# LIS-TU-Berlin/SVN-ICP

Measured on NVIDIA B200. Metric: scans/sec at 1000 particles (64-beam ~120k-pt synthetic scan, K=100, 30 SVN iterations), higher is better.
Workload: dtype f32 geometry / f64 reduction+Stein

## Files before the change

include/svnicp_b200.h:

```cpp
#ifndef SVNICP_B200_H
#define SVNICP_B200_H

#include <stdint.h>

#ifdef __cplusplus
extern "C" {
#endif

#define SVNICP_B200_ABI_VERSION 2

typedef struct svnicp_handle_t *svnicp_handle;

typedef enum {
  SVNICP_OK = 0,
  SVNICP_ERR_INVALID = -1,
  SVNICP_ERR_NO_DEVICE = -2,
  SVNICP_ERR_CUDA = -3,
  SVNICP_ERR_NCCL = -4,
  SVNICP_ERR_OOM = -5
} svnicp_status;

#define SVNICP_ALIGN_SUCCESS 1
#define SVNICP_NO_OPTIMIZER 2

#define SVNICP_CLASS_SVNICP 0
#define SVNICP_CLASS_SVGDICP 1

typedef struct {
  int32_t iterations;
  int32_t use_minibatch;
  int32_t batch_size;
  double lr;
  double max_dist;
  int32_t normalize_cloud;
  char optimizer[16];
  int32_t check_early_stop;
  int32_t convergence_steps;
  double convergence_threshold;
  int32_t KNN_count;
  int32_t SVN_full_grad;
  int32_t use_weight_mean;
  double grid_cell;
  int32_t debug_corr;
  int32_t flags;
  int32_t gn_stages;
  int32_t gn_smem_kb;
} svnicp_params;

#define SVNICP_FLAG_NO_PARTICLE_SORT 1
#define SVNICP_FLAG_FILTER_FULL 2
#define SVNICP_FLAG_NCCL_GATHER 8
#define SVNICP_FLAG_DEBUG_SYNC 32
#define SVNICP_FLAG_WATCHDOG 64
#define SVNICP_FLAG_NO_GRAPH 128
#define SVNICP_FLAG_FORCE_GRAPH 256
#define SVNICP_FLAG_REUSE_STATS 16

void svnicp_default_params(svnicp_params *p);

int svnicp_abi_version(void);

int svnicp_create(svnicp_handle *out, const svnicp_params *params, int particle_count, const double *init_pose,
                  int class_type, int device);
void svnicp_destroy(svnicp_handle h);
const char *svnicp_last_error(svnicp_handle h);

int svnicp_set_stream(svnicp_handle h, void *cuda_stream);

int svnicp_nccl_unique_id(void *id128);
int svnicp_init_sharding(svnicp_handle h, const void *unique_id128, int rank, int n_ranks);

int svnicp_add_cloud(svnicp_handle h, const double *source, int64_t n_s, int source_on_device, const double *target,
                     int64_t n_t, int target_on_device, const double *init_pose);

int svnicp_set_initial_mean(svnicp_handle h, const double R0[9], const double t0[3]);

int svnicp_align(svnicp_handle h);

int svnicp_get_transformation(svnicp_handle h, double out6[6]);
int svnicp_get_distribution(svnicp_handle h, double out6[6]);
int svnicp_get_cov_matrix(svnicp_handle h, double out36[36]);
int svnicp_get_particles(svnicp_handle h, double *out_6xP);
int svnicp_get_particle_weight(svnicp_handle h, double *out_P);
int svnicp_get_particle_history(svnicp_handle h, float *out_Ix6xP, int32_t *rows );
int svnicp_get_runtime(svnicp_handle h, double out3[3]);
int svnicp_set_k(svnicp_handle h, int k);
int svnicp_set_threshold(svnicp_handle h, double max_dist);

int svnicp_initialize_particles(int particle_count, const double ub[6], const double lb[6], uint64_t seed, double *out_6xP);
int svnicp_initialize_particles_gaussian(int particle_count, const double cov_diag[6], uint64_t seed, double *out_6xP);

int svnicp_iterations_done(svnicp_handle h, int32_t *out);
int svnicp_get_candidates(svnicp_handle h, int32_t *out_idx , float *out_rel_xyz );
int svnicp_get_source_f32(svnicp_handle h, float *out_xyz);
int svnicp_get_correspondences(svnicp_handle h, float *out_transforms, int32_t *out_idx, uint8_t *out_mask);
int svnicp_get_gn_system(svnicp_handle h, double *out_H, double *out_b, double *out_x);
int svnicp_get_stein(svnicp_handle h, double *out_delta, double *out_bandwidth);
int svnicp_get_prune_stats(svnicp_handle h, double *out_mean_kept, int32_t *rows);
int svnicp_get_timing(svnicp_handle h, double out4[4]);
int svnicp_get_slice(svnicp_handle h, int32_t *lo, int32_t *hi);
int svnicp_set_profiling(svnicp_handle h, int on);
int svnicp_get_phase_times(svnicp_handle h, double out8[8]);
int svnicp_get_scan_info(svnicp_handle h, int64_t out8[8]);
int svnicp_get_tail_stamps(svnicp_handle h, double out8[8]);
int svnicp_get_launch_count(svnicp_handle h, int64_t *out);

typedef struct svnicp_batch_t *svnicp_batch;
int svnicp_batch_create(svnicp_batch *out, const svnicp_params *params, int n_streams, int particle_count, const double *init_pose,
                        int device);
// ... 36 lines not shown
```

svn_icp_b200/__init__.py:

```python
from __future__ import annotations

import ctypes as C
import dataclasses
import os

import numpy as np

_HERE = os.path.dirname(os.path.abspath(__file__))
LIB_PATH = os.environ.get("SVNICP_B200_LIB") or os.path.join(_HERE, "lib", "libsvnicp_b200.so")

ALIGN_SUCCESS = 1
NO_OPTIMIZER = 2
CLASS_SVNICP = 0
CLASS_SVGDICP = 1


class SvnIcpError(RuntimeError):
    pass


class _CParams(C.Structure):
    _fields_ = [("iterations", C.c_int32), ("use_minibatch", C.c_int32), ("batch_size", C.c_int32), ("lr", C.c_double),
                ("max_dist", C.c_double), ("normalize_cloud", C.c_int32), ("optimizer", C.c_char * 16),
                ("check_early_stop", C.c_int32), ("convergence_steps", C.c_int32), ("convergence_threshold", C.c_double),
                ("KNN_count", C.c_int32), ("SVN_full_grad", C.c_int32), ("use_weight_mean", C.c_int32),
                ("grid_cell", C.c_double), ("debug_corr", C.c_int32), ("flags", C.c_int32), ("gn_stages", C.c_int32),
                ("gn_smem_kb", C.c_int32)]


FLAG_NO_PARTICLE_SORT = 1
FLAG_FILTER_FULL = 2
FLAG_NCCL_GATHER = 8
FLAG_REUSE_STATS = 16
FLAG_DEBUG_SYNC = 32
FLAG_WATCHDOG = 64
FLAG_NO_GRAPH = 128
FLAG_FORCE_GRAPH = 256


@dataclasses.dataclass
class SteinICPParam:
    iterations: int = 50
    use_minibatch: bool = False
    batch_size: int = 50
    lr: float = 0.02
    max_dist: float = 1.0
    normalize_cloud: bool = True
    optimizer: str = "Adam"
    check_early_stop: bool = False
    convergence_steps: int = 5
    convergence_threshold: float = 1e-5
    KNN_count: int = 100
    SVN_full_grad: bool = True
    grid_cell: float = 0.0
    debug_corr: bool = False
    flags: int = 0
    gn_stages: int = 0
    gn_smem_kb: int = 0


@dataclasses.dataclass
class ParticleWeightOpt:
    use_weight_mean: bool = False


_lib = None

EXPORTS = [
    "svnicp_abi_version", "svnicp_default_params", "svnicp_create", "svnicp_destroy", "svnicp_last_error", "svnicp_set_stream",
    "svnicp_nccl_unique_id", "svnicp_init_sharding", "svnicp_add_cloud", "svnicp_set_initial_mean", "svnicp_align",
    "svnicp_get_transformation", "svnicp_get_distribution", "svnicp_get_cov_matrix", "svnicp_get_particles",
    "svnicp_get_particle_weight", "svnicp_get_particle_history", "svnicp_get_runtime", "svnicp_set_k", "svnicp_set_threshold",
    "svnicp_initialize_particles", "svnicp_initialize_particles_gaussian", "svnicp_iterations_done", "svnicp_get_candidates",
    "svnicp_get_source_f32", "svnicp_get_correspondences", "svnicp_get_gn_system", "svnicp_get_stein", "svnicp_get_prune_stats",
    "svnicp_get_timing", "svnicp_get_slice", "svnicp_get_launch_count", "svnicp_set_profiling", "svnicp_get_phase_times",
    "svnicp_get_scan_info", "svnicp_get_tail_stamps",
    "svnicp_map_create", "svnicp_map_destroy", "svnicp_map_last_error", "svnicp_map_clear", "svnicp_map_add_cloud", "svnicp_map_get",
    "svnicp_map_download", "svnicp_map_size",
    "svnicp_pre_create", "svnicp_pre_destroy", "svnicp_pre_last_error", "svnicp_pre_crop", "svnicp_pre_downsample_uniform",
    "svnicp_pre_to_f64", "svnicp_pre_download", "svnicp_pre_deskew", "svnicp_pose_compose",
    "svnicp_batch_create", "svnicp_batch_destroy", "svnicp_batch_last_error", "svnicp_batch_size", "svnicp_batch_stream", "svnicp_batch_align",
]


def load_library() -> C.CDLL:
    global _lib
    if _lib is None:
        if not os.path.exists(LIB_PATH):
            raise SvnIcpError(f"{LIB_PATH} not found: build it with `python -m svn_icp_b200.build` "
                              "(there is no CPU or PyTorch fallback for this path)")
# ... 498 lines not shown
```

svn_icp_b200/csrc/cand_build.cu:

```cuda
#include "common.cuh"
#include "kernels.h"

namespace svn {

constexpr unsigned long long EMPTY_KEY = 0xffffffffffffffffull;
constexpr int RING_MAX = 6;
constexpr int KNN_WARPS = 4;
#ifndef SVN_KNN_CAP
#define SVN_KNN_CAP 512
#endif
constexpr int KNN_CAP = SVN_KNN_CAP;
constexpr int KNN_BINS = 64;

struct Ent {
  double d;
  int pos;
  int idx;
};

__device__ __forceinline__ int cell_of(double x, double inv_cell) { return (int)floor(x * inv_cell); }
__device__ __forceinline__ unsigned long long pack_key(int cx, int cy, int cz) {
  return ((unsigned long long)(unsigned)(cx + (1 << 20)) & 0x1fffffull) << 42 |
         ((unsigned long long)(unsigned)(cy + (1 << 20)) & 0x1fffffull) << 21 |
         ((unsigned long long)(unsigned)(cz + (1 << 20)) & 0x1fffffull);
// ... 322 lines not shown
        SVN_KNN_RELIEVE()
      }
    }
#undef SVN_KNN_RELIEVE
    if (done) {
      int *hist = s_hist[warp];
      hist[lane] = 0;
      hist[lane + 32] = 0;
      __syncwarp();
      const double scale = (double)KNN_BINS / rs2_done;
      for (int i = lane; i < count; i += 32) {
        const double d = buf[i].d;
        if (d < rs2_done) atomicAdd(&hist[min(KNN_BINS - 1, (int)(d * scale))], 1);
      }
      __syncwarp();
      const int h0 = hist[2 * lane], h1 = hist[2 * lane + 1];
      int incl = h0 + h1;
#pragma unroll
      for (int o = 1; o < 32; o <<= 1) {
        const int v = __shfl_up_sync(0xffffffffu, incl, o);
        if (lane >= o) incl += v;
      }
      const int before = incl - h0 - h1;
      int tbin = KNN_BINS;
      if (before < K && before + h0 >= K) tbin = 2 * lane;
      else if (before + h0 < K && incl >= K) tbin = 2 * lane + 1;
#pragma unroll
      for (int o = 16; o > 0; o >>= 1) tbin = min(tbin, __shfl_xor_sync(0xffffffffu, tbin, o));
      int m_out = 0;
      for (int i0 = 0; i0 < count; i0 += 32) {
        const int i = i0 + lane;
        Ent e;
        bool keep = false;
        if (i < count) {
          e = buf[i];
          keep = (e.d < rs2_done) && (min(KNN_BINS - 1, (int)(e.d * scale)) <= tbin);
        }
        const unsigned m = __ballot_sync(0xffffffffu, keep);
        __syncwarp();
        if (keep) buf[m_out + __popc(m & lt_mask)] = e;
        m_out += __popc(m);
        __syncwarp();
      }
      count = m_out;
    }
    count = warp_compact(buf, count, K, &tau);

    for (int k = lane; k < K; k += 32) {
      const double *m;
      int gi;
      if (k < count) { m = sxyz + 3 * (size_t)buf[k].pos; gi = buf[k].idx; }
      else { m = tgt; gi = 0; }
      const float cx = __double2float_rn(m[0] - q[0]), cy = __double2float_rn(m[1] - q[1]), cz = __double2float_rn(m[2] - q[2]);
      const double nrm = sqrt((double)cx * cx + (double)cy * cy + (double)cz * cz);
      const float w = (k < count) ? __double2float_rd(nrm * (1.0 - 1e-6)) : INFINITY;
      cand[(size_t)b * K + k] = make_float4(cx, cy, cz, w);
      if (cand_idx) cand_idx[(size_t)b * K + k] = gi;
    }
    __syncwarp();
  }
}

static inline int cdiv(long long a, long long b) { return (int)((a + b - 1) / b); }

size_t knn_smem_bytes() { return (size_t)KNN_WARPS * KNN_CAP * sizeof(Ent); }

int launch_cand_build(const CandBuildArgs &a, cudaStream_t st) {
  int launches = 0;
  const int T = 256;
  k_q0<<<cdiv(a.n_pad, T), T, 0, st>>>(a.src64, a.n_s, a.sc, a.q0, a.sp, a.n_pad); launches++;
  k_grid_clear<<<cdiv(a.table_size, T), T, 0, st>>>(a.keys, a.counts, a.fill, a.table_size, a.cursor); launches++;
  k_grid_count<<<cdiv(a.n_t, T), T, 0, st>>>(a.tgt64, a.n_t, 1.0 / a.cell, a.keys, a.counts, a.pt_slot, (unsigned)(a.table_size - 1)); launches++;
  k_grid_alloc<<<cdiv(a.table_size, T), T, 0, st>>>(a.counts, a.starts, a.table_size, a.cursor); launches++;
  k_grid_scatter<<<cdiv(a.n_t, T), T, 0, st>>>(a.tgt64, a.n_t, a.pt_slot, a.starts, a.fill, a.sxyz, a.sidx); launches++;
  if (knn_smem_bytes() > 48 * 1024) cudaFuncSetAttribute(k_knn, cudaFuncAttributeMaxDynamicSharedMemorySize, (int)knn_smem_bytes());
  int grid = cdiv(a.row_hi - a.row_lo, KNN_WARPS);
  const int max_grid = a.sm_count * 12;
  if (grid > max_grid) grid = max_grid;
  if (grid < 1) grid = 1;
  k_knn<<<grid, KNN_WARPS * 32, knn_smem_bytes(), st>>>(a.q0, a.row_lo, a.row_hi, a.tgt64, a.n_t, a.sxyz, a.sidx, a.keys, a.starts, a.counts,
                                                         (unsigned)(a.table_size - 1), a.cell, a.K, a.cand, a.cand_idx, a.fallback_count);
  launches++;
  return launches;
}

}
```

svn_icp_b200/csrc/capi.cu:

```cuda
#include <cuda_runtime.h>
#include <dlfcn.h>
#include <math.h>
#include <nccl.h>
#include <stdarg.h>
#include <stdio.h>
#include <time.h>
#include <stdlib.h>
#include <string.h>

#include <algorithm>
#include <cmath>
#include <string>
#include <vector>

#include "../../include/svnicp_b200.h"
#include "common.cuh"
#include "kernels.h"

using namespace svn;

static thread_local std::string g_create_error;

struct NcclApi {
  void *lib = nullptr;
// ... 666 lines not shown
    h->launches += launch_stats_svgd(sa0, nullptr, st);
    CU(cudaGetLastError());
    CU(cudaMemcpyAsync(h->h_stats, h->stats.p, 48 * sizeof(double), cudaMemcpyDeviceToHost, st));
    CU(cudaMemcpyAsync(h->h_particles, h->particles.p, (size_t)6 * h->P * sizeof(double), cudaMemcpyDeviceToHost, st));
    CU(cudaStreamSynchronize(st));
    memset(h->h_ctrl, 0, sizeof(Ctrl));
    memset(h->h_kept, 0, ((size_t)I + 2) * sizeof(unsigned long long));
    h->iters_done = 0;
    h->enqueued_iters = 0;
    h->ms_setup = h->ms_iter = h->ms_epi = h->ms_total = 0;
    h->aligned = true;
    S.special = true;
    return SVNICP_NO_OPTIMIZER;
  }

  CU(cudaEventRecord(h->ev[0], st));
  CandBuildArgs cb;
  cb.src64 = h->src64.p; cb.tgt64 = h->tgt64.p;
  cb.n_s = (int)h->n_s; cb.n_pad = h->n_pad; cb.n_t = (int)h->n_t; cb.K = h->K;
  cb.sc = h->sc;
  cb.cell = h->prm.grid_cell > 0 ? h->prm.grid_cell : 1.5;
  cb.q0 = h->q0.p; cb.sp = h->sp.p;
  cb.keys = h->keys.p; cb.counts = h->counts.p; cb.starts = h->starts.p; cb.fill = h->fill.p; cb.pt_slot = h->pt_slot.p;
  cb.cursor = h->misc.p; cb.fallback_count = h->misc.p + 1;
  size_t table = 1024;
  while (table < (size_t)2 * h->n_t) table <<= 1;
  cb.table_size = (int)table;
  cb.sxyz = h->sxyz.p; cb.sidx = h->sidx.p; cb.cand = h->cand.p; cb.cand_idx = h->prm.debug_corr ? h->cand_idx.p : nullptr;
  cb.sm_count = h->sm_count;
  cb.row_lo = h->rank * h->rows_per_rank;
  cb.row_hi = cb.row_lo + h->rows_per_rank < (int)h->n_s ? cb.row_lo + h->rows_per_rank : (int)h->n_s;
  if (cb.row_hi < cb.row_lo) cb.row_hi = cb.row_lo;
  h->launches += launch_cand_build(cb, st);
  if (h->n_ranks > 1) {
    const size_t blk = (size_t)h->rows_per_rank * h->K;
    NC(g_nccl.AllGather(h->cand.p + (size_t)h->rank * blk, h->cand.p, blk * 4, ncclFloat, h->comm, st));
    if (h->prm.debug_corr) NC(g_nccl.AllGather(h->cand_idx.p + (size_t)h->rank * blk, h->cand_idx.p, blk, ncclInt32, h->comm, st));
  }
  CU(cudaGetLastError());
  CU(cudaEventRecord(h->ev[1], st));

  IterArgs &ia = S.ia;
  memset(&ia, 0, sizeof(ia));
  ia.n_s = (int)h->n_s; ia.n_pad = h->n_pad; ia.K = h->K; ia.Kp = h->Kp; ia.cand_idx = h->prm.debug_corr ? h->cand_idx.p : nullptr;
  ia.P = h->P; ia.p_lo = h->p_lo; ia.P_l = h->P_l;
  ia.sc = h->sc;
  ia.max_dist = (float)h->max_dist;
  ia.sp = h->sp.p; ia.cand = h->cand.p; ia.clist = h->clist.p; ia.hdr = h->hdr.p;
  ia.R = h->R.p; ia.t = h->t.p; ia.xf = h->xf.p; ia.dnorm = h->dnorm.p; ia.part = h->part.p; ia.rec = h->rec; ia.rec_stride = h->rec_stride; ia.ctrl = h->ctrl.p;
  ia.TB = h->TB; ia.stages = h->stages; ia.n_slices = h->n_slices; ia.n_pgroups = h->n_pgroups; ia.PG = h->PG; ia.RG = h->RG;
  ia.gn_lag = (h->prm.gn_stages >> 8) ? (h->prm.gn_stages >> 8) : ((h->stages >= 4) ? 2 : 1);
  ia.gn_smem = h->gn_smem; ia.sm_count = h->sm_count; ia.svn_full_grad = h->prm.SVN_full_grad;
  ia.first_order = svgd ? 1 : 0;
  ia.dbg_idx = h->prm.debug_corr ? h->dbg_idx.p : nullptr;
  ia.dbg_mask = h->prm.debug_corr ? h->dbg_mask.p : nullptr;

  SteinArgs &sa = S.sa;
  memset(&sa, 0, sizeof(sa));
  sa.P = h->P; sa.p_lo = h->p_lo; sa.P_l = h->P_l; sa.I = I;
  sa.svn_full_grad = h->prm.SVN_full_grad; sa.check_early_stop = h->prm.check_early_stop;
  sa.lr = h->prm.lr; sa.threshold = h->prm.convergence_threshold;
  sa.rec = h->rec; sa.rec_stride = h->rec_stride; sa.xs = h->xs.p; sa.delta = h->delta.p; sa.dnorm = h->dnorm.p; sa.R = h->R.p; sa.t = h->t.p;
  sa.Hbar_inv = h->Hbar_inv.p; sa.hist = h->hist.p; sa.history = h->history.p; sa.ctrl = h->ctrl.p;
  sa.stats = h->stats.p; sa.particles = h->particles.p; sa.sm_count = h->sm_count;
  sa.kept_hist = h->kept_hist.p;
  sa.prep_scratch_d = h->prep_scratch_d.p;
  sa.prep_scratch_i = h->prep_scratch_i.p;
  sa.stamps = h->profile ? h->stamps.p : nullptr;
  const bool overlap = S.overlap = !svgd && (h->n_ranks == 1 || h->peer_mode);
  S.pt = h->pt;
  S.seq0 = h->seq;
  S.use_graph = overlap && h->n_ranks == 1 && !h->profile && !h->prm.debug_corr && !h->graph_off &&
                !(h->prm.flags & (SVNICP_FLAG_DEBUG_SYNC | SVNICP_FLAG_NO_GRAPH)) &&
                ((h->prm.flags & SVNICP_FLAG_FORCE_GRAPH) || (!h->prm.check_early_stop && I >= 16 && (double)h->n_s * (double)h->P_l <= 1.0e7));

  if (h->profile)
    while (h->prof_events.size() < (size_t)I * 7) {
      cudaEvent_t pe;
      CU(cudaEventCreate(&pe));
      h->prof_events.push_back(pe);
    }
  if (!svgd) {
    const double *x_src = (realign && h->n_ranks > 1) ? h->rec + (size_t)(h->iters_done & 1) * h->rec_stride : nullptr;
    h->launches += launch_prep(ia, st, 1, x_src);
    if (overlap) CU(cudaEventRecord(h->ev_x, st));
  }
  S.e = 0;
  S.enqueue_done = I <= 0;
  return SVNICP_OK;
}

static int align_step(svnicp_handle h, AlignState &S) {
  ALIGN_LOCALS
  const int LAG = 3;
  const int e = S.e;
    if (h->prm.check_early_stop && e >= LAG) {
      CU(cudaEventSynchronize(h->iter_events[e - LAG]));
      if (h->h_stop[e - LAG]) { S.enqueue_done = true; return SVNICP_OK; }
    }
#define PROF(k)                                                                                          \
  do {                                                                                                   \
    if (h->profile) CU(cudaEventRecord(h->prof_events[(size_t)e * 7 + (k)], st));                        \
    if (h->prm.flags & SVNICP_FLAG_DEBUG_SYNC) {                                                         \
      fprintf(stderr, "[svnicp] iteration %d: before phase %d ...", e, (k));                             \
      fflush(stderr);                                                                                    \
      const cudaError_t e1__ = cudaStreamSynchronize(st), e2__ = cudaStreamSynchronize(hs);              \
// ... 532 lines not shown
```

svn_icp_b200/csrc/iter_kernels.cu:

```cuda
#include "common.cuh"
#include "kernels.h"
#include "ptx.cuh"

namespace svn {

__global__ void __launch_bounds__(1024) k_prep(IterArgs a, int all_x, const double *x_src) {
  if (a.ctrl->stop) return;
  __shared__ double s_red[32][12];
  __shared__ float s_center[12];
  __shared__ double s_max[32][2];
  __shared__ int s_env[PRUNE_BINS];
  __shared__ int s_nan;
  const int tid = threadIdx.x, lane = tid & 31, warp = tid >> 5;
  const double *R0 = a.sc.R0;
  double acc[12];
#pragma unroll
  for (int i = 0; i < 12; i++) acc[i] = 0.0;
  for (int l = tid; l < a.P_l; l += blockDim.x) {
    const int p = a.p_lo + l;
    double R[9], t[3], w[3];
#pragma unroll
    for (int i = 0; i < 9; i++) R[i] = a.R[9 * (size_t)p + i];
#pragma unroll
    for (int i = 0; i < 3; i++) t[i] = a.t[3 * (size_t)p + i];
// ... 319 lines not shown
__device__ __forceinline__ float sqrt_approx(float x) {
  float r;
  asm("sqrt.approx.ftz.f32 %0, %1;" : "=f"(r) : "f"(x));
  return r;
}
__device__ __forceinline__ float rcp_approx(float x) {
  float r;
  asm("rcp.approx.ftz.f32 %0, %1;" : "=f"(r) : "f"(x));
  return r;
}

typedef unsigned long long f2;
__device__ __forceinline__ f2 pk(float a, float b) { f2 r; asm("mov.b64 %0, {%1, %2};" : "=l"(r) : "f"(a), "f"(b)); return r; }
__device__ __forceinline__ float lo(f2 v) { float a; asm("{ .reg .f32 t; mov.b64 {%0, t}, %1; }" : "=f"(a) : "l"(v)); return a; }
__device__ __forceinline__ float hi(f2 v) { float a; asm("{ .reg .f32 t; mov.b64 {t, %0}, %1; }" : "=f"(a) : "l"(v)); return a; }
__device__ __forceinline__ f2 bc(float s) { return pk(s, s); }
__device__ __forceinline__ f2 fma2(f2 a, f2 b, f2 c) { f2 r; asm("fma.rn.f32x2 %0, %1, %2, %3;" : "=l"(r) : "l"(a), "l"(b), "l"(c)); return r; }
__device__ __forceinline__ f2 add2(f2 a, f2 b) { f2 r; asm("add.rn.f32x2 %0, %1, %2;" : "=l"(r) : "l"(a), "l"(b)); return r; }
__device__ __forceinline__ f2 sub2(f2 a, f2 b) { f2 r; asm("sub.rn.f32x2 %0, %1, %2;" : "=l"(r) : "l"(a), "l"(b)); return r; }
__device__ __forceinline__ f2 mul2(f2 a, f2 b) { f2 r; asm("mul.rn.f32x2 %0, %1, %2;" : "=l"(r) : "l"(a), "l"(b)); return r; }
__device__ __forceinline__ f2 neg2(f2 a) { return pk(-lo(a), -hi(a)); }
__device__ __forceinline__ f2 sel2(bool p0, bool p1, f2 a, f2 b) { return pk(p0 ? lo(a) : lo(b), p1 ? hi(a) : hi(b)); }
__device__ __forceinline__ f2 min4_2(f2 a, f2 b, f2 c, f2 d) {
  return pk(fminf(fminf(lo(a), lo(b)), fminf(lo(c), lo(d))), fminf(fminf(hi(a), hi(b)), fminf(hi(c), hi(d))));
}

__device__ __noinline__ void gn_dbg_tap(const IterArgs &a, int row, int l, float qx, float qy, float qz, float ex, float ey, float ez, bool valid) {
  const float4 *full_row = a.cand + (size_t)row * a.K;
  const float wx_ = __fsub_rn(qx, ex), wy_ = __fsub_rn(qy, ey), wz_ = __fsub_rn(qz, ez);
  int slot = 0;
  float bd_ = INFINITY;
  for (int kk = 0; kk < a.K; kk++) {
    const float4 f = full_row[kk];
    const float dd_ = fabsf(f.x - wx_) + fabsf(f.y - wy_) + fabsf(f.z - wz_);
    if (dd_ < bd_) { bd_ = dd_; slot = kk; }
  }
  a.dbg_idx[(size_t)l * a.n_s + row] = a.cand_idx[(size_t)row * a.K + slot];
  a.dbg_mask[(size_t)l * a.n_s + row] = valid ? 1 : 0;
}

__device__ __forceinline__ void gn_recover(const float4 *e, int bk, float qx, float qy, float qz, float best, float &ex, float &ey, float &ez) {
  const float4 c0 = e[bk], c1 = e[bk + 1], c2 = e[bk + 2], c3 = e[bk + 3];
#define SVN_D1(C, T)                                                                                      \
  const float T##x = __fsub_rn(qx, (C).x), T##y = __fsub_rn(qy, (C).y), T##z = __fsub_rn(qz, (C).z);       \
  const float T##d = __fmaf_rn(T##z, T##z, __fmaf_rn(T##y, T##y, __fmul_rn(T##x, T##x)));
  SVN_D1(c0, u) SVN_D1(c1, v) SVN_D1(c2, w) SVN_D1(c3, z)
#undef SVN_D1
  (void)zd;
  const bool h0 = ud == best, h1 = vd == best, h2 = wd == best;
  ex = h0 ? ux : h1 ? vx : h2 ? wx : zx;
  ey = h0 ? uy : h1 ? vy : h2 ? wy : zy;
  ez = h0 ? uz : h1 ? vz : h2 ? wz : zz;
  if (best == INFINITY) { ex = ux; ey = uy; ez = uz; }
}

template <bool DBG, bool UNI, bool FIRST>
__global__ void __launch_bounds__(GN_THREADS, 1) k_gn(IterArgs a) {
  if (a.ctrl->stop) return;
  extern __shared__ __align__(128) unsigned char smem[];
  const int TB = a.TB, Kp = a.Kp, S = a.stages;
  const size_t stage_bytes = gn_stage_bytes(TB, Kp);
  uint64_t *full = reinterpret_cast<uint64_t *>(smem + (size_t)S * stage_bytes);
  uint64_t *empty = full + S;
  const int tid = threadIdx.x, warp = tid >> 5, lane = tid & 31;
  const int n_tiles = a.n_pad / TB;
  const int slice = blockIdx.x, n_slices = gridDim.x;
  const int n_my = (slice < n_tiles) ? (n_tiles - slice + n_slices - 1) / n_slices : 0;
  const size_t hdr_off = (size_t)TB * Kp * 16, msk_off = hdr_off + (size_t)TB * 16;

  if (tid == 0) {
    for (int s = 0; s < S; s++) { mbar_init(full + s, 1); mbar_init(empty + s, GN_CONSUMERS / 32); }
    fence_barrier_init();
  }
  __syncthreads();

  constexpr int NW = GN_CONSUMERS / 32;
  auto tile_cnt = [&](int j) -> int {
    return (lane < TB) ? (__float_as_int(__ldg(&a.hdr[(size_t)(slice + j * n_slices) * TB + lane].w)) >> 16) : 0;
  };
  auto tile_issue = [&](int j, int cnt) {
    const int s = j % S;
    const int row0 = (slice + j * n_slices) * TB;
    unsigned char *st = smem + (size_t)s * stage_bytes;
    const unsigned m2 = __ballot_sync(0xffffffffu, cnt == 2), m4 = __ballot_sync(0xffffffffu, cnt == 4), ml = __ballot_sync(0xffffffffu, cnt > 4);
    const int bytes = cnt * 16;
    SVN_CHECK(a.ctrl, cnt >= 0 && cnt <= Kp && row0 + TB <= a.n_pad, 1);
    int total = bytes;
#pragma unroll
    for (int o = 16; o > 0; o >>= 1) total += __shfl_xor_sync(0xffffffffu, total, o);
    total += TB * 16;
    if (lane == 0) {
      unsigned *msk = reinterpret_cast<unsigned *>(st + msk_off);
      msk[0] = m2; msk[1] = m4; msk[2] = ml;
      mbar_expect_tx(full + s, (uint32_t)total);
    }
    __syncwarp();
    if (lane < TB && cnt > 0) bulk_g2s(st + (size_t)lane * Kp * 16, a.clist + (size_t)(row0 + lane) * Kp, (uint32_t)bytes, full + s);
    if (lane == 0) bulk_g2s(st + hdr_off, a.hdr + row0, (uint32_t)(TB * 16), full + s);
  };
  const int LAG = (a.gn_lag < S) ? a.gn_lag : 1, AHEAD = S - LAG;
  for (int j = 0; j < AHEAD && j < n_my; j++)
    if (warp == j % NW) tile_issue(j, tile_cnt(j));
  int cnt_pref = (warp == 0 && AHEAD < n_my) ? tile_cnt(AHEAD) : 0;

  const int PG = a.PG, RG = a.RG;
  const int pl = tid % PG, rg = tid / PG;
// ... 80 lines not shown
      unsigned m2 = msk[0] & rgmask, m4 = msk[1] & rgmask, ml = msk[2] & rgmask;
      rows_in_acc += __popc(m2 | m4 | ml);
#define SVN_ROW2(SV, CA, CB)                                                                                            \
  {                                                                                                                     \
    const float4 sv = (SV);                                                                                             \
    SVN_QUERY                                                                                                           \
    SVN_DIST(CA, u) SVN_DIST(CB, v)                                                                                     \
                                 \
    const bool p0 = lo(vd) < lo(ud), p1 = hi(vd) < hi(ud);                                                              \
    const f2 best = sel2(p0, p1, vd, ud), ex = sel2(p0, p1, vx, ux), ey = sel2(p0, p1, vy, uy), ez = sel2(p0, p1, vz, uz); \
    SVN_ACCUM(true)                                                                                                     \
  }
      while (m2 & (m2 - 1)) {
        const int r0 = __ffs(m2) - 1;
        m2 &= m2 - 1;
        const int r1 = __ffs(m2) - 1;
        m2 &= m2 - 1;
        const float4 sv0 = hdr[r0], sv1 = hdr[r1];
        const float4 *e0 = lists + r0 * Kp, *e1 = lists + r1 * Kp;
        const float4 c00 = e0[0], c01 = e0[1], c10 = e1[0], c11 = e1[1];
        { const int r = r0; (void)r; SVN_ROW2(sv0, c00, c01) }
        { const int r = r1; (void)r; SVN_ROW2(sv1, c10, c11) }
      }
      if (m2) {
        const int r = __ffs(m2) - 1;
        const float4 *e0 = lists + r * Kp;
        const float4 sv0 = hdr[r], c00 = e0[0], c01 = e0[1];
        SVN_ROW2(sv0, c00, c01)
      }
#undef SVN_ROW2
      while (m4) {
        const int r = __ffs(m4) - 1;
        m4 &= m4 - 1;
        const float4 sv = hdr[r];
        const float4 *e = lists + r * Kp;
        const float4 c0 = e[0], c1 = e[1], c2 = e[2], c3 = e[3];
        SVN_QUERY
        SVN_DIST(c0, u) SVN_DIST(c1, v) SVN_DIST(c2, w) SVN_DIST(c3, z)
        const bool p10 = lo(vd) < lo(ud), p11 = hi(vd) < hi(ud), p30 = lo(zd) < lo(wd), p31 = hi(zd) < hi(wd);
        const f2 m01 = sel2(p10, p11, vd, ud), m23 = sel2(p30, p31, zd, wd);
        const f2 e01x = sel2(p10, p11, vx, ux), e01y = sel2(p10, p11, vy, uy), e01z = sel2(p10, p11, vz, uz);
        const f2 e23x = sel2(p30, p31, zx, wx), e23y = sel2(p30, p31, zy, wy), e23z = sel2(p30, p31, zz, wz);
        const bool p0 = lo(m23) < lo(m01), p1 = hi(m23) < hi(m01);
        const f2 best = sel2(p0, p1, m23, m01), ex = sel2(p0, p1, e23x, e01x), ey = sel2(p0, p1, e23y, e01y), ez = sel2(p0, p1, e23z, e01z);
        SVN_ACCUM(true)
      }
      while (ml) {
        const int r = __ffs(ml) - 1;
        ml &= ml - 1;
        const float4 sv = hdr[r];
        const float4 *e = lists + r * Kp;
        const int n = __float_as_int(sv.w) >> 16;
        SVN_CHECK(a.ctrl, n > 4 && n <= Kp && (n & 3) == 0 && r < TB, 2);
        float4 c0 = e[0], c1 = e[1], c2 = e[2], c3 = e[3];
        SVN_QUERY
        float best0, best1;
        int bk0 = 0, bk1 = 0;
        {
          SVN_DIST(c0, u) SVN_DIST(c1, v) SVN_DIST(c2, w) SVN_DIST(c3, z)
          const f2 m_ = min4_2(ud, vd, wd, zd);
          best0 = lo(m_); best1 = hi(m_);
          if (!(best0 == best0)) best0 = INFINITY;
          if (!(best1 == best1)) best1 = INFINITY;
        }
        const f2 qq = fma2(qz, qz, fma2(qy, qy, mul2(qx, qx)));
        const f2 qn = fma2(pk(sqrt_approx(lo(qq)), sqrt_approx(hi(qq))), bc(1.00001f), bc(1e-7f));
        for (int k0 = 4; k0 < n; k0 += 4) {
          c0 = e[k0]; c1 = e[k0 + 1]; c2 = e[k0 + 2]; c3 = e[k0 + 3];
          const f2 tt = sub2(bc(c0.w), qn);
          const f2 tb = mul2(mul2(tt, tt), bc(0.99999f));
          const bool done = (lo(tt) > 0.f) && (lo(tb) > best0) && (hi(tt) > 0.f) && (hi(tb) > best1);
          if (UNI) { if (__all_sync(0xffffffffu, done)) break; }
          else { if (done) break; }
          SVN_DIST(c0, u) SVN_DIST(c1, v) SVN_DIST(c2, w) SVN_DIST(c3, z)
          const f2 m_ = min4_2(ud, vd, wd, zd);
          if (lo(m_) < best0) { best0 = lo(m_); bk0 = k0; }
          if (hi(m_) < best1) { best1 = hi(m_); bk1 = k0; }
        }
        SVN_CHECK(a.ctrl, bk0 >= 0 && bk0 + 3 < n && bk1 >= 0 && bk1 + 3 < n, 3);
        float ex0, ey0, ez0, ex1, ey1, ez1;
        gn_recover(e, bk0, lo(qx), lo(qy), lo(qz), best0, ex0, ey0, ez0);
        gn_recover(e, bk1, hi(qx), hi(qy), hi(qz), best1, ex1, ey1, ez1);
        const f2 best = pk(best0, best1), ex = pk(ex0, ex1), ey = pk(ey0, ey1), ez = pk(ez0, ez1);
        SVN_ACCUM(true)
      }
      if (rows_in_acc >= GN_FLUSH_ROWS) {
#pragma unroll
        for (int j = 0; j < NACC; j++) { dacc[j * GN_CONSUMERS] = add2(dacc[j * GN_CONSUMERS], acc[j]); acc[j] = 0; }
        rows_in_acc = 0;
        if (++flushes2 >= GN_FLUSH2 && active) {
#pragma unroll
          for (int j = 0; j < NACC; j++) {
            const f2 d = dacc[j * GN_CONSUMERS];
            out[j] = (wrote ? out[j] : 0.0) + (double)lo(d);
            if (active1) out[NACC + j] = (wrote ? out[NACC + j] : 0.0) + (double)hi(d);
            dacc[j * GN_CONSUMERS] = 0;
          }
          wrote = true;
          flushes2 = 0;
        }
      }
    }
    __syncwarp();
    if (lane == 0) mbar_arrive(empty + s);
  }
#undef SVN_QUERY
#undef SVN_DIST
#undef SVN_ACCUM
  if (active) {
#pragma unroll
    for (int j = 0; j < NACC; j++) {
      const f2 d = dacc[j * GN_CONSUMERS];
      out[j] = (wrote ? out[j] : 0.0) + ((double)lo(d) + (double)lo(acc[j]));
      if (active1) out[NACC + j] = (wrote ? out[NACC + j] : 0.0) + ((double)hi(d) + (double)hi(acc[j]));
    }
  }
}

__global__ void __launch_bounds__(FIN_WARPS * 32) k_finalize(IterArgs a, PeerTable pt, unsigned seq_h) {
  Ctrl *ctl = a.ctrl;
  if (ctl->stop) return;
  __shared__ double s_out[REC];
  __shared__ int s_last;
  const int l = blockIdx.x;
  double v[NACC];
  gn_sum_partials(a, l, v);
  const int p = a.p_lo + l;
  SVN_CHECK(ctl, l < a.P_l && p < a.P && (size_t)(p + 1) * REC <= a.rec_stride, 20);
  const size_t buf_off = (size_t)(ctl->iter & 1) * a.rec_stride;
  if (threadIdx.x == 0) {
    const double *R0 = a.sc.R0;
    double Rp[9], Rt[9];
#pragma unroll
    for (int i = 0; i < 9; i++) Rp[i] = a.R[9 * (size_t)p + i];
#pragma unroll
// ... 144 lines not shown
```

svn_icp_b200/csrc/kernels.h:

```cpp
#pragma once
#include <cuda_runtime.h>
#include <stdint.h>
#include "common.cuh"

namespace svn {

struct CandBuildArgs {
  const double *src64, *tgt64;
  int n_s, n_pad, n_t, K;
  int row_lo, row_hi;
  ScanConst sc;
  double cell;
  double *q0;
  float4 *sp;
  unsigned long long *keys;
  int *counts, *starts, *fill, *pt_slot, *cursor;
  int table_size;
  double *sxyz;
  int *sidx;
  float4 *cand;
  int *cand_idx;
  int *fallback_count;
  int sm_count;
};
int launch_cand_build(const CandBuildArgs &a, cudaStream_t st);
size_t knn_smem_bytes();

struct IterArgs {
  int n_s, n_pad, K;
  int Kp;
  const int *cand_idx;
  int P;
  int p_lo, P_l;
  ScanConst sc;
  float max_dist;
  const float4 *sp, *cand;
  float4 *clist;
  float4 *hdr;
  const float4 *clist_prev;
  const int *cbase_prev;
  const float4 *ball_prev;
  int *cbase;
  float4 *ball;
  const unsigned long long *kept_hist;
  double *R, *t;
  float *xf;
  double *dnorm;
  double *part;
  double *rec;
  size_t rec_stride;
  Ctrl *ctrl;
  int TB, stages, n_slices, n_pgroups, PG, RG;
  int gn_lag;
  size_t gn_smem;
  int sm_count;
  int svn_full_grad;
  int first_order;
  int32_t *dbg_idx;
  uint8_t *dbg_mask;
};
#ifdef __CUDACC__
constexpr int FIN_WARPS = 8;
__host__ __device__ inline int fin_rows(const IterArgs &a) { return a.n_slices * (a.RG < a.TB ? a.RG : a.TB); }
inline int fin_threads(const IterArgs &a) { return fin_rows(a) > 512 ? FIN_WARPS * 32 : 128; }
__device__ __forceinline__ void gn_sum_partials(const IterArgs &a, int l, double v[NACC]) {
  __shared__ double s_fin[FIN_WARPS][NACC];
  const int lane = threadIdx.x & 31, w = threadIdx.x >> 5, nw = blockDim.x >> 5;
  const int nrows = fin_rows(a);
  const int j16 = lane & 15, half = lane >> 4;
  double s0 = 0.0, s1 = 0.0, s2 = 0.0, s3 = 0.0;
  const int step = 2 * nw;
  int r = half + 2 * w;
  for (; r + 3 * step < nrows; r += 4 * step) {
    s0 += a.part[((size_t)r * a.P_l + l) * NACC + j16];
    s1 += a.part[((size_t)(r + step) * a.P_l + l) * NACC + j16];
    s2 += a.part[((size_t)(r + 2 * step) * a.P_l + l) * NACC + j16];
    s3 += a.part[((size_t)(r + 3 * step) * a.P_l + l) * NACC + j16];
  }
  for (; r < nrows; r += step) s0 += a.part[((size_t)r * a.P_l + l) * NACC + j16];
  double s = (s0 + s1) + (s2 + s3);
  s += __shfl_down_sync(0xffffffffu, s, 16);
  if (lane < NACC) s_fin[w][lane] = s;
  __syncthreads();
#pragma unroll
  for (int j = 0; j < NACC; j++) {
    double t = s_fin[0][j];
    for (int ww = 1; ww < nw; ww++) t += s_fin[ww][j];
    v[j] = t;
  }
}
#endif
int launch_prep(const IterArgs &a, cudaStream_t st, int all_x, const double *x_src);
int launch_filter(const IterArgs &a, cudaStream_t st);
int launch_gn(const IterArgs &a, cudaStream_t st);
int launch_finalize(const IterArgs &a, const PeerTable &pt, unsigned seq_h, cudaStream_t st);
void init_iter_kernels();
__host__ __device__ inline size_t gn_stage_bytes(int TB, int K) { return ((size_t)TB * K * 16 + (size_t)TB * 16 + 16 + 127) & ~(size_t)127; }
constexpr int GN_CONSUMERS = 512;
constexpr int GN_THREADS = GN_CONSUMERS;
__host__ __device__ inline size_t gn_dacc_offset(int TB, int K, int S) { return (gn_stage_bytes(TB, K) * S + 2 * (size_t)S * 8 + 127) & ~(size_t)127; }
__host__ __device__ inline size_t gn_smem_bytes(int TB, int K, int S) { return gn_dacc_offset(TB, K, S) + (size_t)NACC * GN_CONSUMERS * 8; }

struct SteinArgs {
  int P, p_lo, P_l, I;
  int svn_full_grad, check_early_stop;
  double lr, threshold;
  double *rec;
  size_t rec_stride;
  double *xs;
  double *delta;
  double *dnorm;
  double *R, *t;
  double *Hbar_inv;
  unsigned *hist;
  float *history;
  Ctrl *ctrl;
  double *stats;
  double *particles;
  unsigned long long *kept_hist;
  double *prep_scratch_d;
  int *prep_scratch_i;
  double *stamps;
  int sm_count;
};
int launch_head(const SteinArgs &a, const PeerTable &pt, unsigned seq_x, int epilogue, cudaStream_t st);
int launch_tail(const SteinArgs &a, const IterArgs &ia, const PeerTable &pt, unsigned seq_h, unsigned seq_x_out, cudaStream_t st);
int launch_decide(const SteinArgs &a, cudaStream_t st, int epilogue);
int launch_median(const SteinArgs &a, cudaStream_t st);
int launch_stats(const SteinArgs &a, int parity_from_ctrl, cudaStream_t st);
int launch_align_reset(Ctrl *ctrl, double *opt_state, size_t n_opt, cudaStream_t st);
int launch_init_particles(double *R, double *t, const double *init_pose_dev, int P, double *dnorm, int p_lo, int P_l, Ctrl *ctrl,
                          cudaStream_t st);


enum { SVGD_OPT_ADAM = 0, SVGD_OPT_RMSPROP = 1, SVGD_OPT_SGD = 2, SVGD_OPT_ADAGRAD = 3 };
struct SvgdArgs {
  int P, p_lo, P_l;
  int optimizer;
  double lr;
  double *pose6;
  double *prev;
  double *opt_state;
};
int launch_svgd_init(const SvgdArgs &s, const double *init_pose_dev, double *R, double *t, double *dnorm, Ctrl *ctrl, cudaStream_t st);
int launch_finalize_first(const IterArgs &a, const SvgdArgs &s, cudaStream_t st);
int launch_svgd_rec(double *rec, const double *src6, const double *dnorm, int lo, int n, int dn_off, cudaStream_t st);
int launch_stein_first(const SteinArgs &a, cudaStream_t st);
int launch_update_opt(const SteinArgs &a, const SvgdArgs &s, int step, cudaStream_t st);
int launch_stats_svgd(const SteinArgs &a, double *prev_out, cudaStream_t st);

}
```

Before: 35.85.

## Screen GN candidates with dot-product bound and resolve exact nearest in fp32

Candidate weights now store half the squared norm instead of the norm, so the nearest-neighbour search in the GN kernel can rank candidates by the linear form w - q·c, which needs fewer FLOPs than a full squared distance. Groups of four whose screened value lies within an error margin of the running minimum are recorded in a bitmask, and the exact distance is recomputed only for those groups in gn_resolve. The early-exit bound is rewritten to match the new weights. A new flag restores the old exact scan, and the screened path is only enabled for K up to 128. The risk is extra bookkeeping and divergence in the resolve step, plus a change in tie and precision behaviour.

```diff
diff --git a/include/svnicp_b200.h b/include/svnicp_b200.h
--- a/include/svnicp_b200.h
+++ b/include/svnicp_b200.h
@@ -55,6 +55,7 @@
 #define SVNICP_FLAG_NO_GRAPH 128
 #define SVNICP_FLAG_FORCE_GRAPH 256
 #define SVNICP_FLAG_REUSE_STATS 16
+#define SVNICP_FLAG_GN_EXACT_SCAN 512
 
 void svnicp_default_params(svnicp_params *p);
 
diff --git a/svn_icp_b200/__init__.py b/svn_icp_b200/__init__.py
--- a/svn_icp_b200/__init__.py
+++ b/svn_icp_b200/__init__.py
@@ -36,6 +36,7 @@
 FLAG_WATCHDOG = 64
 FLAG_NO_GRAPH = 128
 FLAG_FORCE_GRAPH = 256
+FLAG_GN_EXACT_SCAN = 512
 
 
 @dataclasses.dataclass
diff --git a/svn_icp_b200/csrc/cand_build.cu b/svn_icp_b200/csrc/cand_build.cu
--- a/svn_icp_b200/csrc/cand_build.cu
+++ b/svn_icp_b200/csrc/cand_build.cu
@@ -398,8 +398,7 @@
       if (k < count) { m = sxyz + 3 * (size_t)buf[k].pos; gi = buf[k].idx; }
       else { m = tgt; gi = 0; }
       const float cx = __double2float_rn(m[0] - q[0]), cy = __double2float_rn(m[1] - q[1]), cz = __double2float_rn(m[2] - q[2]);
-      const double nrm = sqrt((double)cx * cx + (double)cy * cy + (double)cz * cz);
-      const float w = (k < count) ? __double2float_rd(nrm * (1.0 - 1e-6)) : INFINITY;
+      const float w = (k < count) ? __double2float_rn(0.5 * ((double)cx * cx + (double)cy * cy + (double)cz * cz)) : INFINITY;
       cand[(size_t)b * K + k] = make_float4(cx, cy, cz, w);
       if (cand_idx) cand_idx[(size_t)b * K + k] = gi;
     }
diff --git a/svn_icp_b200/csrc/capi.cu b/svn_icp_b200/csrc/capi.cu
--- a/svn_icp_b200/csrc/capi.cu
+++ b/svn_icp_b200/csrc/capi.cu
@@ -742,6 +742,7 @@
   ia.gn_lag = (h->prm.gn_stages >> 8) ? (h->prm.gn_stages >> 8) : ((h->stages >= 4) ? 2 : 1);
   ia.gn_smem = h->gn_smem; ia.sm_count = h->sm_count; ia.svn_full_grad = h->prm.SVN_full_grad;
   ia.first_order = svgd ? 1 : 0;
+  ia.gn_screen = (!(h->prm.flags & SVNICP_FLAG_GN_EXACT_SCAN) && h->Kp <= GN_SCREEN_MAX_KP) ? 1 : 0;
   ia.dbg_idx = h->prm.debug_corr ? h->dbg_idx.p : nullptr;
   ia.dbg_mask = h->prm.debug_corr ? h->dbg_mask.p : nullptr;
 
diff --git a/svn_icp_b200/csrc/iter_kernels.cu b/svn_icp_b200/csrc/iter_kernels.cu
--- a/svn_icp_b200/csrc/iter_kernels.cu
+++ b/svn_icp_b200/csrc/iter_kernels.cu
@@ -395,6 +395,42 @@
   ey = h0 ? uy : h1 ? vy : h2 ? wy : zy;
   ez = h0 ? uz : h1 ? vz : h2 ? wz : zz;
   if (best == INFINITY) { ex = ux; ey = uy; ez = uz; }
+}
+
+constexpr float GN_SCREEN_REL = 0x1p-18f, GN_SCREEN_ABS = 0x1p-100f, GN_SCREEN_BIG = 0x1p100f;
+__device__ __forceinline__ f2 abs2(f2 a) { return pk(fabsf(lo(a)), fabsf(hi(a))); }
+
+__device__ __forceinline__ void gn_resolve(const float4 *e, unsigned mask, float qx, float qy, float qz, float &best, float &ex, float &ey, float &ez) {
+  if (!(mask & (mask - 1))) {
+    const int k = mask ? 4 * (__ffs(mask) - 1) : 0;
+    const float4 c0 = e[k], c1 = e[k + 1], c2 = e[k + 2], c3 = e[k + 3];
+#define SVN_D1(C, T)                                                                                      \
+  const float T##x = __fsub_rn(qx, (C).x), T##y = __fsub_rn(qy, (C).y), T##z = __fsub_rn(qz, (C).z);       \
+  const float T##d = __fmaf_rn(T##z, T##z, __fmaf_rn(T##y, T##y, __fmul_rn(T##x, T##x)));
+    SVN_D1(c0, u) SVN_D1(c1, v) SVN_D1(c2, w) SVN_D1(c3, z)
+#undef SVN_D1
+    best = fminf(fminf(ud, vd), fminf(wd, zd));
+    const bool h0 = ud == best, h1 = vd == best, h2 = wd == best;
+    ex = h0 ? ux : h1 ? vx : h2 ? wx : zx;
+    ey = h0 ? uy : h1 ? vy : h2 ? wy : zy;
+    ez = h0 ? uz : h1 ? vz : h2 ? wz : zz;
+    if (mask && best < INFINITY) return;
+    best = INFINITY;
+    if (k == 0) { ex = ux; ey = uy; ez = uz; return; }
+  }
+  ex = __fsub_rn(qx, e[0].x); ey = __fsub_rn(qy, e[0].y); ez = __fsub_rn(qz, e[0].z);
+  best = INFINITY;
+  while (mask) {
+    const int k = 4 * (__ffs(mask) - 1);
+    mask &= mask - 1;
+#pragma unroll
+    for (int j = 0; j < 4; j++) {
+      const float4 c = e[k + j];
+      const float ux = __fsub_rn(qx, c.x), uy = __fsub_rn(qy, c.y), uz = __fsub_rn(qz, c.z);
+      const float ud = __fmaf_rn(uz, uz, __fmaf_rn(uy, uy, __fmul_rn(ux, ux)));
+      if (ud < best) { best = ud; ex = ux; ey = uy; ez = uz; }
+    }
+  }
 }
 
 template <bool DBG, bool UNI, bool FIRST>
@@ -581,35 +617,70 @@
         const float4 *e = lists + r * Kp;
         const int n = __float_as_int(sv.w) >> 16;
         SVN_CHECK(a.ctrl, n > 4 && n <= Kp && (n & 3) == 0 && r < TB, 2);
-        float4 c0 = e[0], c1 = e[1], c2 = e[2], c3 = e[3];
         SVN_QUERY
-        float best0, best1;
-        int bk0 = 0, bk1 = 0;
-        {
-          SVN_DIST(c0, u) SVN_DIST(c1, v) SVN_DIST(c2, w) SVN_DIST(c3, z)
-          const f2 m_ = min4_2(ud, vd, wd, zd);
-          best0 = lo(m_); best1 = hi(m_);
-          if (!(best0 == best0)) best0 = INFINITY;
-          if (!(best1 == best1)) best1 = INFINITY;
+        const f2 qq = fma2(qz, qz, fma2(qy, qy, mul2(qx, qx)));
+        const f2 nqn = fma2(pk(sqrt_approx(lo(qq)), sqrt_approx(hi(qq))), bc(-0.70712f), bc(-1e-7f));
+        float best0, best1, ex0, ey0, ez0, ex1, ey1, ez1;
+        if (a.gn_screen) {
+          const int nt = __float_as_int(sv.w) & 0xffff;
+          SVN_CHECK(a.ctrl, nt > 0 && nt <= n && n <= GN_SCREEN_MAX_KP, 5);
+          const f2 wq = fma2(qq, bc(0.5f), bc(e[nt - 1].w));
+          f2 eps = fma2(wq, bc(GN_SCREEN_REL), bc(GN_SCREEN_ABS));
+          eps = pk(lo(wq) <= GN_SCREEN_BIG ? lo(eps) : INFINITY, hi(wq) <= GN_SCREEN_BIG ? hi(eps) : INFINITY);
+          const f2 e2 = add2(eps, eps), nqe = fma2(eps, bc(-2.f), mul2(qq, bc(-0.5f)));
+#define SVN_SCREEN(C) fma2(neg2(qx), bc((C).x), fma2(neg2(qy), bc((C).y), fma2(neg2(qz), bc((C).z), bc((C).w))))
+          f2 V;
+          unsigned mk0, mk1, bit = 1u;
+          {
+            const float4 c0 = e[0], c1 = e[1], c2 = e[2], c3 = e[3];
+            const f2 m_ = min4_2(SVN_SCREEN(c0), SVN_SCREEN(c1), SVN_SCREEN(c2), SVN_SCREEN(c3));
+            mk0 = (lo(m_) == lo(m_)) ? 1u : 0u;
+            mk1 = (hi(m_) == hi(m_)) ? 1u : 0u;
+            V = pk(fminf(INFINITY, lo(m_)), fminf(INFINITY, hi(m_)));
+          }
+          for (const float4 *p = e + 4, *pe = e + n; p < pe; p += 4) {
+            const float4 c0 = p[0], c1 = p[1], c2 = p[2], c3 = p[3];
+            const f2 tt = fma2(bc(sqrt_approx(c0.w)), bc(0.99999f), nqn);
+            const f2 tb = fma2(tt, abs2(tt), nqe);
+            const bool done = (lo(tb) > lo(V)) && (hi(tb) > hi(V));
+            if (UNI) { if (__all_sync(0xffffffffu, done)) break; }
+            else { if (done) break; }
+            const f2 m_ = min4_2(SVN_SCREEN(c0), SVN_SCREEN(c1), SVN_SCREEN(c2), SVN_SCREEN(c3));
+            const f2 D = sub2(m_, V);
+            bit += bit;
+            if (lo(D) <= lo(e2)) mk0 = ((lo(D) < -lo(e2)) ? 0u : mk0) | bit;
+            if (hi(D) <= hi(e2)) mk1 = ((hi(D) < -hi(e2)) ? 0u : mk1) | bit;
+            V = pk(fminf(lo(V), lo(m_)), fminf(hi(V), hi(m_)));
+          }
+#undef SVN_SCREEN
+          gn_resolve(e, mk0, lo(qx), lo(qy), lo(qz), best0, ex0, ey0, ez0);
+          gn_resolve(e, mk1, hi(qx), hi(qy), hi(qz), best1, ex1, ey1, ez1);
+        } else {
+          int bk0 = 0, bk1 = 0;
+          {
+            const float4 c0 = e[0], c1 = e[1], c2 = e[2], c3 = e[3];
+            SVN_DIST(c0, u) SVN_DIST(c1, v) SVN_DIST(c2, w) SVN_DIST(c3, z)
+            const f2 m_ = min4_2(ud, vd, wd, zd);
+            best0 = lo(m_); best1 = hi(m_);
+            if (!(best0 == best0)) best0 = INFINITY;
+            if (!(best1 == best1)) best1 = INFINITY;
+          }
+          for (int k0 = 4; k0 < n; k0 += 4) {
+            const float4 c0 = e[k0], c1 = e[k0 + 1], c2 = e[k0 + 2], c3 = e[k0 + 3];
+            const f2 tt = fma2(bc(sqrt_approx(c0.w)), bc(0.99999f), nqn);
+            const f2 tb = mul2(mul2(tt, abs2(tt)), bc(1.99998f));
+            const bool done = (lo(tb) > best0) && (hi(tb) > best1);
+            if (UNI) { if (__all_sync(0xffffffffu, done)) break; }
+            else { if (done) break; }
+            SVN_DIST(c0, u) SVN_DIST(c1, v) SVN_DIST(c2, w) SVN_DIST(c3, z)
+            const f2 m_ = min4_2(ud, vd, wd, zd);
+            if (lo(m_) < best0) { best0 = lo(m_); bk0 = k0; }
+            if (hi(m_) < best1) { best1 = hi(m_); bk1 = k0; }
+          }
+          SVN_CHECK(a.ctrl, bk0 >= 0 && bk0 + 3 < n && bk1 >= 0 && bk1 + 3 < n, 3);
+          gn_recover(e, bk0, lo(qx), lo(qy), lo(qz), best0, ex0, ey0, ez0);
+          gn_recover(e, bk1, hi(qx), hi(qy), hi(qz), best1, ex1, ey1, ez1);
         }
-        const f2 qq = fma2(qz, qz, fma2(qy, qy, mul2(qx, qx)));
-        const f2 qn = fma2(pk(sqrt_approx(lo(qq)), sqrt_approx(hi(qq))), bc(1.00001f), bc(1e-7f));
-        for (int k0 = 4; k0 < n; k0 += 4) {
-          c0 = e[k0]; c1 = e[k0 + 1]; c2 = e[k0 + 2]; c3 = e[k0 + 3];
-          const f2 tt = sub2(bc(c0.w), qn);
-          const f2 tb = mul2(mul2(tt, tt), bc(0.99999f));
-          const bool done = (lo(tt) > 0.f) && (lo(tb) > best0) && (hi(tt) > 0.f) && (hi(tb) > best1);
-          if (UNI) { if (__all_sync(0xffffffffu, done)) break; }
-          else { if (done) break; }
-          SVN_DIST(c0, u) SVN_DIST(c1, v) SVN_DIST(c2, w) SVN_DIST(c3, z)
-          const f2 m_ = min4_2(ud, vd, wd, zd);
-          if (lo(m_) < best0) { best0 = lo(m_); bk0 = k0; }
-          if (hi(m_) < best1) { best1 = hi(m_); bk1 = k0; }
-        }
-        SVN_CHECK(a.ctrl, bk0 >= 0 && bk0 + 3 < n && bk1 >= 0 && bk1 + 3 < n, 3);
-        float ex0, ey0, ez0, ex1, ey1, ez1;
-        gn_recover(e, bk0, lo(qx), lo(qy), lo(qz), best0, ex0, ey0, ez0);
-        gn_recover(e, bk1, hi(qx), hi(qy), hi(qz), best1, ex1, ey1, ez1);
         const f2 best = pk(best0, best1), ex = pk(ex0, ex1), ey = pk(ey0, ey1), ez = pk(ez0, ez1);
         SVN_ACCUM(true)
       }
diff --git a/svn_icp_b200/csrc/kernels.h b/svn_icp_b200/csrc/kernels.h
--- a/svn_icp_b200/csrc/kernels.h
+++ b/svn_icp_b200/csrc/kernels.h
@@ -56,6 +56,7 @@
   int sm_count;
   int svn_full_grad;
   int first_order;
+  int gn_screen;
   int32_t *dbg_idx;
   uint8_t *dbg_mask;
 };
@@ -98,6 +99,7 @@
 __host__ __device__ inline size_t gn_stage_bytes(int TB, int K) { return ((size_t)TB * K * 16 + (size_t)TB * 16 + 16 + 127) & ~(size_t)127; }
 constexpr int GN_CONSUMERS = 512;
 constexpr int GN_THREADS = GN_CONSUMERS;
+constexpr int GN_SCREEN_MAX_KP = 128;
 __host__ __device__ inline size_t gn_dacc_offset(int TB, int K, int S) { return (gn_stage_bytes(TB, K) * S + 2 * (size_t)S * 8 + 127) & ~(size_t)127; }
 __host__ __device__ inline size_t gn_smem_bytes(int TB, int K, int S) { return gn_dacc_offset(TB, K, S) + (size_t)NACC * GN_CONSUMERS * 8; }
 
```

Result: slower. 34.00, median of 6 (-5.2%).
